# CompVis/behavior-driven-video-synthesis

Hardware: AMD Instinct MI355X
Metric: frames/sec VUnet 256x256 bs=16 fwd+bwd (higher is better)
Workload: dtype f32 (operands scaled by a power of two and split into 2 fp16 terms, 3 partial products on fp16 MFMA, fp32 accumulate; weight gradients and uncovered layers: 3 bf16 terms / 6 products, fp32-input MFMA, fp32 VALU); 1 GPU; Human3.6m shape_and_pose_net VunetAlter 256x256 per-GPU bs=16 fwd+bwd, VGG19 perceptual + KL loss, fused Adam, dropout 0.05, regressor side loop off, seeded-synthetic VGG19 weights, rasterised synthetic stickmen; global_batch=16, parallelism=dp1, conv_precision=h2, hip_streams=4, hip_graph=True, graph_settle_steps=7, rccl_world_size=1, dp_backend=none

## Files before the change

### behavior_driven_video_synthesis_amd/csrc/conv_wgrad_direct.hip

```cpp
#include <type_traits>

#include "common.h"
#include "split_h2.h"

struct WgradDirectArgs {
  vunet_wgrad_desc d;
  const float* x1;
  const float* x2;
  const float* dy;
  float* slabs;
  float* dshift;
  const float* amax_x;
  const float* amax_x2;
  const float* amax_dy;
  int Ctot, Coutp, ncot, noct, ops;
  int opr, opi;
  InAct in1, in2;
};

typedef uint32_t wd_u32x4 __attribute__((ext_vector_type(4)));
typedef float wd_f32x4 __attribute__((ext_vector_type(4)));

template <int S, bool W4, int T>
__device__ __forceinline__ void wgrad_direct_body(WgradDirectArgs& a, const int bx, const int by) {
  inact_resolve(a.in1);
  inact_resolve(a.in2);
  static_assert(T != 3 || !W4, "the kernel-row split is for maps >= 8 wide");
  constexpr int R = (T == 1 || T == 3) ? 1 : (W4 ? S + 3 : 3);
  constexpr int L = T == 1 ? 8 : (W4 ? 4 * S + 2 : 8 * S + 2);
  const vunet_wgrad_desc& d = a.d;
  const int tid = threadIdx.x, lane = tid & 63, wave = tid >> 6;
  const int j = lane & 31, h = lane >> 5;
  const int unit0 = bx * 4 + wave;
  const int krow = T == 3 ? unit0 % 3 : 0;
  const int unit = T == 3 ? unit0 / 3 : unit0;
  const int cot = unit % a.ncot, split = unit / a.ncot;
  const int ci0 = by * 32;
  const int H = d.Hs, W = d.Ws, HW = H * W, HoWo = d.Ho * d.Wo;

  float sx, sdy, descale, descale2;
  {
    __shared__ float redm[8];
    const float4 px = h2_amax4(a.amax_x, a.amax_x2, tid), pd = reinterpret_cast<const float4*>(a.amax_dy)[tid];
    float mx = wave_max(fmaxf(fmaxf(px.x, px.y), fmaxf(px.z, px.w)));
    float md = wave_max(fmaxf(fmaxf(pd.x, pd.y), fmaxf(pd.z, pd.w)));
    if (lane == 0) { redm[wave] = mx; redm[4 + wave] = md; }
    __syncthreads();
    mx = fmaxf(fmaxf(redm[0], redm[1]), fmaxf(redm[2], redm[3]));
    md = fmaxf(fmaxf(redm[4], redm[5]), fmaxf(redm[6], redm[7]));
    if (a.in1.thresh) mx *= a.in1.keep_scale;
    const int ex = h2_scale_exp(mx), ed = h2_scale_exp(md);
    sx = h2_pow2(ex);
    sdy = h2_pow2(ed);
    h2_pow2_pair(-(ex + ed), descale, descale2);
  }
  if (split >= d.nsplit) return;

  const int ci = ci0 + j;
  const bool ci_ok = ci < a.Ctot;
  const bool second = ci_ok && ci >= d.C1;
  const float* __restrict__ xs = second ? a.x2 : a.x1;
  const int Cs = second ? d.C2 : d.C1;
  const int cl = ci_ok ? (second ? ci - d.C1 : ci) : 0;
  InAct ia = a.in1;
  ia.seed = second ? a.in2.seed : a.in1.seed;
  const int co = cot * 32 + j;
  const bool co_ok = co < d.Cout;

  f32x16 acc[T];
#pragma unroll
  for (int t = 0; t < T; ++t)
#pragma unroll
    for (int r = 0; r < 16; ++r) acc[t][r] = 0.f;
  float dsum = 0.f;

  const int pro_form = in_act_form_of(a.in1);
  const int o_begin = split * a.ops, o_end = min(o_begin + a.ops, a.noct);
#pragma unroll(T == 1 ? 4 : 1)
  for (int o2 = o_begin; o2 < o_end; o2 += 2) {
    const int o = o2 + h;
    const bool ov = o < o_end;
    const int oc = ov ? o : o_begin;
    const int n = oc / a.opi, rem = oc - n * a.opi;
    int r0, c0;
    if (T == 1) { r0 = 0; c0 = rem * 8; }
    else if (W4) { r0 = rem * 2; c0 = 0; }
    else { r0 = rem / a.opr; c0 = (rem - r0 * a.opr) * 8; }

    h2_f16x8 Ah, Al;
    {
      const float* dp = a.dy + (size_t)(n * d.Cout + (co_ok ? co : 0)) * HoWo + (T == 1 ? c0 : r0 * d.Wo + c0);
      wd_f32x4 d0 = *reinterpret_cast<const wd_f32x4*>(dp), d1 = *reinterpret_cast<const wd_f32x4*>(dp + 4);
      if (!(ov && co_ok)) { d0 = wd_f32x4{0.f, 0.f, 0.f, 0.f}; d1 = d0; }
      dsum += ((d0[0] + d0[1]) + (d0[2] + d0[3])) + ((d1[0] + d1[1]) + (d1[2] + d1[3]));
      uint32_t ah[4], al[4];
      h2_split2_nat(d0[0] * sdy, d0[1] * sdy, ah[0], al[0]);
      h2_split2_nat(d0[2] * sdy, d0[3] * sdy, ah[1], al[1]);
      h2_split2_nat(d1[0] * sdy, d1[1] * sdy, ah[2], al[2]);
      h2_split2_nat(d1[2] * sdy, d1[3] * sdy, ah[3], al[3]);
      Ah = h2_frag(ah[0], ah[1], ah[2], ah[3]);
      Al = h2_frag(al[0], al[1], al[2], al[3]);
    }

    float seg[R][L];
    auto stage = [&](auto pro_c) {
      constexpr int PRO = decltype(pro_c)::value;
      const uint32_t cbase = (uint32_t)(n * Cs + cl) * (uint32_t)HW;
      const float* xp = xs + cbase;
#pragma unroll
      for (int rr = 0; rr < R; ++rr) {
        const int ih = T == 1 ? 0 : S * r0 - 1 + rr + krow;
        const bool rok = ov && ci_ok && (T == 1 || (unsigned)ih < (unsigned)H);
        const int ihc = rok ? ih : 0;
        const float sxr = rok ? sx : 0.f;
        if (T == 1) {
          const uint32_t off = (uint32_t)c0;
          const wd_f32x4 v0 = *reinterpret_cast<const wd_f32x4*>(xp + off), v1 = *reinterpret_cast<const wd_f32x4*>(xp + off + 4);
#pragma unroll
          for (int e = 0; e < 8; ++e) {
            const float t_ = e < 4 ? v0[e] : v1[e - 4];
            seg[rr][e] = in_act_form<PRO>(ia, rok ? t_ : 0.f, cbase + off + e) * sxr;
          }
        } else {
          constexpr int NV = (L - 2) / 4;
          const uint32_t off = (uint32_t)(ihc * W + S * c0);
          wd_f32x4 v[NV];
#pragma unroll
          for (int q = 0; q < NV; ++q) v[q] = *reinterpret_cast<const wd_f32x4*>(xp + off + 4 * q);
          const bool lok = rok && c0 > 0, hok = rok && S == 1 && S * c0 + 4 * NV < W;
          const float lv = xp[lok ? off - 1 : off];
          const float hv = xp[hok ? off + 4 * NV : off];
          seg[rr][0] = in_act_form<PRO>(ia, lok ? lv : 0.f, cbase + off - 1) * (lok ? sx : 0.f);
#pragma unroll
          for (int e = 0; e < 4 * NV; ++e)
            seg[rr][1 + e] = in_act_form<PRO>(ia, rok ? v[e >> 2][e & 3] : 0.f, cbase + off + e) * sxr;
          seg[rr][L - 1] = in_act_form<PRO>(ia, hok ? hv : 0.f, cbase + off + 4 * NV) * (hok ? sx : 0.f);
        }
      }
    };
    if (pro_form == 2) stage(std::integral_constant<int, 2>{});
    else if (pro_form == 1) stage(std::integral_constant<int, 1>{});
    else if (pro_form == 0) stage(std::integral_constant<int, 0>{});
    else stage(std::integral_constant<int, 3>{});

#pragma unroll
    for (int t = 0; t < T; ++t) {
      const int kh = T == 3 ? 0 : t / 3, kw = t % 3;
      float f[8];
#pragma unroll
      for (int e = 0; e < 8; ++e) {
        if (T == 1) f[e] = seg[0][e];
        else if (W4) f[e] = seg[(e >> 2) * S + kh][(e & 3) * S + kw];
        else f[e] = seg[kh][e * S + kw];
      }
      uint32_t bh[4], bl[4];
      h2_split2_nat(f[0], f[1], bh[0], bl[0]);
      h2_split2_nat(f[2], f[3], bh[1], bl[1]);
      h2_split2_nat(f[4], f[5], bh[2], bl[2]);
      h2_split2_nat(f[6], f[7], bh[3], bl[3]);
      const h2_f16x8 Bh = h2_frag(bh[0], bh[1], bh[2], bh[3]), Bl = h2_frag(bl[0], bl[1], bl[2], bl[3]);
      f32x16 cc = acc[t];
      cc = __builtin_amdgcn_mfma_f32_32x32x16_f16(Ah, Bl, cc, 0, 0, 0);
      cc = __builtin_amdgcn_mfma_f32_32x32x16_f16(Al, Bh, cc, 0, 0, 0);
      cc = __builtin_amdgcn_mfma_f32_32x32x16_f16(Ah, Bh, cc, 0, 0, 0);
      acc[t] = cc;
    }
  }

  const size_t KT = (size_t)(T == 3 ? 9 : T) * a.Ctot;
  float* slab = a.slabs + (size_t)split * a.Coutp * KT;
  if (ci_ok) {
    auto store = [&](auto tc) {
      constexpr int t = decltype(tc)::value;
      const int tap = T == 3 ? krow * 3 + t : t;
#pragma unroll
      for (int r = 0; r < 16; ++r) {
        const int cr = cot * 32 + (r & 3) + 8 * (r >> 2) + 4 * h;
        if (cr < d.Cout) slab[(size_t)cr * KT + (size_t)tap * a.Ctot + ci] = acc[t][r] * descale * descale2;
      }
    };
    store(std::integral_constant<int, 0>{});
    if constexpr (T == 3) {
      store(std::integral_constant<int, 1>{});
      store(std::integral_constant<int, 2>{});
    }
    if constexpr (T == 9) {
      store(std::integral_constant<int, 1>{});
      store(std::integral_constant<int, 2>{});
      store(std::integral_constant<int, 3>{});
      store(std::integral_constant<int, 4>{});
      store(std::integral_constant<int, 5>{});
      store(std::integral_constant<int, 6>{});
      store(std::integral_constant<int, 7>{});
      store(std::integral_constant<int, 8>{});
    }
  }
  if (by == 0 && krow == 0) {
    const float tot = dsum + __shfl_xor(dsum, 32, 64);
    if (h == 0 && co < a.Coutp) a.dshift[(size_t)split * a.Coutp + co] = co_ok ? tot : 0.f;
  }
}

template <int S, bool W4, int T>
__global__ __launch_bounds__(256, 2) void conv_wgrad_direct_kernel(const WgradDirectArgs a_in) {
  WgradDirectArgs a = a_in;
  wgrad_direct_body<S, W4, T>(a, (int)blockIdx.x, (int)blockIdx.y);
}

struct S2Lds {
  static constexpr int PITCH = 48;
  static constexpr int XPLANE = 32 * PITCH;
  static constexpr int XBYTES = 3 * 4 * XPLANE;
  static constexpr int DYCOT = 2 * 32 * PITCH;
};

__device__ __forceinline__ wd_f32x4 s2_load4(const float* p) {
  wd_f32x4 v;
  asm volatile("global_load_dwordx4 %0, %1, off" : "=v"(v) : "v"(p) : "memory");
  return v;
}
__device__ __forceinline__ float s2_load1(const float* p) {
  float v;
  asm volatile("global_load_dword %0, %1, off" : "=v"(v) : "v"(p) : "memory");
  return v;
}
template <int N>
__device__ __forceinline__ void s2_wait() {
  static_assert(N >= 0 && N < 64, "vmcnt is six bits");
  asm volatile("s_waitcnt vmcnt(%0)" ::"n"(N) : "memory");
}

template <int NWAVE, int NU, int NCOT>
__global__ __launch_bounds__(64 * NWAVE) void conv_wgrad_s2_kernel(const WgradDirectArgs a_in) {
  WgradDirectArgs a = a_in;
  inact_resolve(a.in1);
  inact_resolve(a.in2);
  constexpr int NTHR = 64 * NWAVE;
  constexpr int NX = (3 * 32 * 8 + NTHR - 1) / NTHR;
  constexpr int NDY = (NCOT * 32 * 4 + NTHR - 1) / NTHR;
  extern __shared__ __attribute__((aligned(16))) unsigned char s2_lds[];
  unsigned char* const xL = s2_lds;
  unsigned char* const dL = s2_lds + S2Lds::XBYTES;
  const vunet_wgrad_desc& d = a.d;
  const int tid = threadIdx.x, lane = tid & 63, wave = tid >> 6;
  const int j = lane & 31, h = lane >> 5;
  const int split = blockIdx.x, ci0 = blockIdx.y * 32;
  const int H = d.Hs, W = d.Ws, HW = H * W, HoWo = d.Ho * d.Wo;
  const int ppr = d.Wo >> 4, ppi = d.Ho * ppr;

  float sx, sdy, descale, descale2;
  {
    __shared__ float redm[2 * NWAVE];
    float mx = 0.f, md = 0.f;
    for (int i = tid; i < 256; i += NTHR) {
      const float4 px = h2_amax4(a.amax_x, a.amax_x2, i), pd = reinterpret_cast<const float4*>(a.amax_dy)[i];
      mx = fmaxf(mx, fmaxf(fmaxf(px.x, px.y), fmaxf(px.z, px.w)));
      md = fmaxf(md, fmaxf(fmaxf(pd.x, pd.y), fmaxf(pd.z, pd.w)));
    }
    mx = wave_max(mx);
    md = wave_max(md);
    if (lane == 0) { redm[wave] = mx; redm[NWAVE + wave] = md; }
    __syncthreads();
    mx = md = 0.f;
#pragma unroll
    for (int w = 0; w < NWAVE; ++w) { mx = fmaxf(mx, redm[w]); md = fmaxf(md, redm[NWAVE + w]); }
    if (a.in1.thresh) mx *= a.in1.keep_scale;
    const int ex = h2_scale_exp(mx), ed = h2_scale_exp(md);
    sx = h2_pow2(ex);
    sdy = h2_pow2(ed);
    h2_pow2_pair(-(ex + ed), descale, descale2);
  }
  const bool second = ci0 >= d.C1;
  const float* __restrict__ xs = second ? a.x2 : a.x1;
  const int Cs = second ? d.C2 : d.C1, cl0 = second ? ci0 - d.C1 : ci0;
  InAct ia = a.in1;
  ia.seed = second ? a.in2.seed : a.in1.seed;
  const int pro_form = in_act_form_of(a.in1);

  const int pairs = d.N * ppi, pps = (pairs + d.nsplit - 1) / d.nsplit;
  const int pb = split * pps, pe = min(pb + pps, pairs);

  const int krow = wave % 3, cotb = wave / 3;
  f32x16 acc[NU][3];
#pragma unroll
  for (int u = 0; u < NU; ++u)
#pragma unroll
    for (int t = 0; t < 3; ++t)
// ... 156 lines not shown
      for (int i = 0; i < NX; ++i) asm volatile("" : "+v"(xv[K_][i]) : : "memory");
#pragma unroll
      for (int i = 0; i < NDY; ++i) asm volatile("" : "+v"(dv[K_][i]) : : "memory");
      asm volatile("" : "+v"(xhalo[K_]) : : "memory");
    }
    lds_barrier();
    if (pro_form == 2) convert(p, std::integral_constant<int, 2>{}, slot_c);
    else if (pro_form == 1) convert(p, std::integral_constant<int, 1>{}, slot_c);
    else if (pro_form == 0) convert(p, std::integral_constant<int, 0>{}, slot_c);
    else convert(p, std::integral_constant<int, 3>{}, slot_c);
    lds_barrier();
    if (p + D < pe) prefetch(p + D, slot_c);
    if (cotb < NCOT) multiply();
  };
  if (pb + 0 < pe) prefetch(pb + 0, std::integral_constant<int, 0>{});
  if constexpr (D == 4) {
    if (pb + 1 < pe) prefetch(pb + 1, std::integral_constant<int, 1>{});
    if (pb + 2 < pe) prefetch(pb + 2, std::integral_constant<int, 2>{});
    if (pb + 3 < pe) prefetch(pb + 3, std::integral_constant<int, 3>{});
  }
  for (int p0 = pb; p0 < pe; p0 += D) {
    step(p0, std::integral_constant<int, 0>{});
    if constexpr (D == 4) {
      if (p0 + 1 < pe) step(p0 + 1, std::integral_constant<int, 1>{});
      if (p0 + 2 < pe) step(p0 + 2, std::integral_constant<int, 2>{});
      if (p0 + 3 < pe) step(p0 + 3, std::integral_constant<int, 3>{});
    }
  }

  const size_t KT = (size_t)9 * a.Ctot;
  float* slab = a.slabs + (size_t)split * a.Coutp * KT;
#pragma unroll
  for (int u = 0; u < NU; ++u) {
    const int cot = cotb + 2 * u;
    if (cot >= NCOT) continue;
#pragma unroll
    for (int t = 0; t < 3; ++t)
#pragma unroll
      for (int r = 0; r < 16; ++r) {
        const int cr = cot * 32 + (r & 3) + 8 * (r >> 2) + 4 * h;
        slab[(size_t)cr * KT + (size_t)(krow * 3 + t) * a.Ctot + ci0 + j] = acc[u][t][r] * descale * descale2;
      }
  }
  if (blockIdx.y == 0) {
#pragma unroll
    for (int i = 0; i < NDY; ++i) {
      const int u = tid + NTHR * i;
      const int q4 = u & 3, co = (u >> 2) & 31, cot = u >> 7;
      float t = dsum[i];
      t += __shfl_xor(t, 1, 64);
      t += __shfl_xor(t, 2, 64);
      if (q4 == 0 && cot < NCOT) a.dshift[(size_t)split * a.Coutp + cot * 32 + co] = t;
    }
  }
}

static bool s2_staged_ok(const vunet_wgrad_desc* d) {
  if (g_vunet_tune[VUNET_TUNE_WGRAD_ROWSPLIT] == 3) return false;
  if (!(d->flags & 2) || (d->flags & 1)) return false;
  if (d->KH != 3 || d->KW != 3 || d->stride != 2 || d->pad != 1) return false;
  if (d->Ws != 2 * d->Wo || d->Hs != 2 * d->Ho || d->Wo % 16) return false;
  if (d->C1 % 32 || d->C2 % 32 || d->Cout % 32) return false;
  const int ncot = d->Cout / 32;
  if (ncot != 1 && ncot != 2 && ncot != 4) return false;
  return (int64_t)d->N * d->Ho * d->Wo > 16384;
}

static int s2_staged_nslabs(const vunet_wgrad_desc* d) {
  const int ncit = (d->C1 + d->C2) / 32, pairs = d->N * d->Ho * (d->Wo / 16);
  int S = 512 / ncit;
  if (S > pairs / 4) S = pairs / 4;
  return S < 1 ? 1 : S;
}

constexpr int WD_MULTI = 12;
struct WgradDirectBatch {
  WgradDirectArgs it[WD_MULTI];
  int start[WD_MULTI + 1];
  int gx[WD_MULTI];
  int n;
};
static_assert(sizeof(WgradDirectBatch) <= 4096, "kernel arguments: 4 KB");
template <int S, bool W4, int T>
__global__ __launch_bounds__(256, 2) void conv_wgrad_direct_multi_kernel(const WgradDirectBatch b) {
  int i = 0;
  while (i + 1 < b.n && (int)blockIdx.x >= b.start[i + 1]) ++i;
  WgradDirectArgs a = b.it[i];
  const int local = (int)blockIdx.x - b.start[i];
  wgrad_direct_body<S, W4, T>(a, local % b.gx[i], local / b.gx[i]);
}

static int direct_class(const vunet_wgrad_desc* d) {
  if (!(d->flags & 2) || (d->flags & 1)) return 0;
  if (d->C1 <= 0 || d->Cout <= 0 || (d->C2 > 0 && d->C1 % 32 != 0)) return 0;
  if (d->Cout < 16 && d->KH == 3) return 0;
  if (d->KH == 1 && d->KW == 1) {
    if (d->stride != 1 || d->pad != 0 || d->Ho != d->Hs || d->Wo != d->Ws || (d->Hs * d->Ws) % 8) return 0;
    return 1;
  }
  if (d->KH != 3 || d->KW != 3 || d->pad != 1 || (d->stride != 1 && d->stride != 2)) return 0;
  if (d->Ho != (d->Hs - 1) / d->stride + 1 || d->Wo != (d->Ws - 1) / d->stride + 1) return 0;
  if (d->Ws % 4) return 0;
  if (d->Wo == 4 && d->Ws == 4 * d->stride && d->Ho % 2 == 0) return d->stride == 1 ? 2 : 3;
  if (d->Wo % 8 == 0 && d->Ws == d->Wo * d->stride) return d->stride == 1 ? 4 : 5;
  return 0;
}

bool vunet_wgrad_direct_applicable(const vunet_wgrad_desc* d) { return direct_class(d) != 0; }

static void direct_geometry(const vunet_wgrad_desc* d, WgradDirectArgs& a) {
  const int cls = direct_class(d);
  a.Ctot = d->C1 + d->C2;
  a.Coutp = (d->Cout + 31) / 32 * 32;
  a.ncot = a.Coutp / 32;
  if (cls == 1) { a.opr = 0; a.opi = d->Hs * d->Ws / 8; }
  else if (cls == 2 || cls == 3) { a.opr = 0; a.opi = d->Ho / 2; }
  else { a.opr = d->Wo / 8; a.opi = d->Ho * a.opr; }
  a.noct = d->N * a.opi;
}

static bool direct_rowsplit(int cls) {
  const int knob = g_vunet_tune[VUNET_TUNE_WGRAD_ROWSPLIT];
  if (knob == 1) return false;
  return cls == 5 || (knob != 4 && cls == 4);
}

int vunet_wgrad_direct_nslabs(const vunet_wgrad_desc* d) {
  if (s2_staged_ok(d)) return s2_staged_nslabs(d);
  WgradDirectArgs a;
  direct_geometry(d, a);
  const int ncit = (a.Ctot + 31) / 32;
  int S = 2048 / (a.ncot * ncit * (direct_rowsplit(direct_class(d)) ? 3 : 1));
  const int by_work = (a.noct + 7) / 8;
  if (S > by_work) S = by_work;
  if (S < 1) S = 1;
  const int cap = d->KH == 1 ? 2048 : 512;
  if (S > cap) S = cap;
  return S;
}

int vunet_wgrad_direct_name(const vunet_wgrad_desc* d, char* name, int len) {
  if (s2_staged_ok(d)) return snprintf(name, len, "conv_wgrad_s2_kernel");
  const int cls = direct_class(d);
  const int S = (cls == 3 || cls == 5) ? 2 : 1, W4 = (cls == 2 || cls == 3), T = cls == 1 ? 1 : (direct_rowsplit(cls) ? 3 : 9);
  return snprintf(name, len, "conv_wgrad_direct_kernel<%d, %s, %d>", S, W4 ? "true" : "false", T);
}

static void direct_fill(const vunet_wgrad_desc* d, const float* x1, const float* x2, const float* dy, float* slabs, float* dshift,
                        const float* amax_x, const float* amax_x2, const float* amax_dy, WgradDirectArgs& a, int& gx, int& gy) {
  a.d = *d;
  a.x1 = x1; a.x2 = x2; a.dy = dy; a.slabs = slabs; a.dshift = dshift; a.amax_x = amax_x; a.amax_x2 = amax_x2; a.amax_dy = amax_dy;
  direct_geometry(d, a);
  a.ops = (a.noct + d->nsplit - 1) / d->nsplit;
  a.ops = (a.ops + 1) & ~1;
  a.in1 = make_inact(d->in_act, d->in_slope, d->drop_p, d->drop_seed);
  a.in2 = make_inact(d->in_act, d->in_slope, d->drop_p, d->drop_seed + 0x9E3779B9u);
  const int units = d->nsplit * a.ncot * (direct_rowsplit(direct_class(d)) ? 3 : 1);
  gx = (units + 3) / 4;
  gy = (a.Ctot + 31) / 32;
}

static int direct_form(const vunet_wgrad_desc* d) {
  const int cls = direct_class(d);
  return cls ? cls * 2 + (direct_rowsplit(cls) ? 1 : 0) : 0;
}

template <int S, bool W4, int T>
static void direct_launch_batch(const WgradDirectBatch& b, hipStream_t st) {
  VUNET_LAUNCH((conv_wgrad_direct_multi_kernel<S, W4, T>), dim3((unsigned)b.start[b.n]), dim3(256), 0, st, b);
}

int vunet_wgrad_direct_launch_multi(const vunet_wgrad_item* items, const int* idx, int cnt, hipStream_t st) {
  if (cnt < 1) return VUNET_OK;
  const int form = direct_form(&items[idx[0]].d);
  if (!form) return VUNET_ERR_UNSUPPORTED;
  for (int at = 0; at < cnt; at += WD_MULTI) {
    WgradDirectBatch b;
    b.n = cnt - at < WD_MULTI ? cnt - at : WD_MULTI;
    b.start[0] = 0;
    for (int k = 0; k < b.n; ++k) {
      const vunet_wgrad_item& it = items[idx[at + k]];
      if (direct_form(&it.d) != form) return VUNET_ERR_ARG;
      if (!it.x1 || !it.dy || !it.slabs || !it.dshift || !it.amax_x || !it.amax_dy || (it.d.C2 > 0 && !it.x2)) return VUNET_ERR_ARG;
      int gx, gy;
      direct_fill(&it.d, it.x1, it.x2, it.dy, it.slabs, it.dshift, it.amax_x, it.amax_x2, it.amax_dy, b.it[k], gx, gy);
      b.gx[k] = gx;
      b.start[k + 1] = b.start[k] + gx * gy;
    }
    for (int k = b.n; k < WD_MULTI; ++k) { b.it[k] = b.it[0]; b.gx[k] = 1; b.start[k + 1] = b.start[b.n]; }
    switch (form) {
      case 2: direct_launch_batch<1, false, 1>(b, st); break;
      case 4: direct_launch_batch<1, true, 9>(b, st); break;
      case 6: direct_launch_batch<2, true, 9>(b, st); break;
      case 8: direct_launch_batch<1, false, 9>(b, st); break;
      case 9: direct_launch_batch<1, false, 3>(b, st); break;
      case 10: direct_launch_batch<2, false, 9>(b, st); break;
      case 11: direct_launch_batch<2, false, 3>(b, st); break;
      default: return VUNET_ERR_UNSUPPORTED;
    }
    const int rc = vunet_check_launch();
    if (rc != VUNET_OK) return rc;
  }
  return VUNET_OK;
}

int vunet_wgrad_direct_form(const vunet_wgrad_desc* d) { return direct_form(d); }

int vunet_wgrad_direct_launch(const vunet_wgrad_desc* d, const float* x1, const float* x2, const float* dy, float* slabs,
                              float* dshift, const float* amax_x, const float* amax_x2, const float* amax_dy, hipStream_t st) {
  const int cls = direct_class(d);
  if (!cls) return VUNET_ERR_UNSUPPORTED;
  WgradDirectArgs a;
  int gx, gy;
  direct_fill(d, x1, x2, dy, slabs, dshift, amax_x, amax_x2, amax_dy, a, gx, gy);
  if (s2_staged_ok(d)) {
    const int ncot = d->Cout / 32;
    dim3 grid((unsigned)d->nsplit, (unsigned)((d->C1 + d->C2) / 32));
    const size_t lds = (size_t)S2Lds::XBYTES + (size_t)ncot * S2Lds::DYCOT;
    if (ncot == 1) VUNET_LAUNCH((conv_wgrad_s2_kernel<3, 1, 1>), grid, dim3(192), lds, st, a);
    else if (ncot == 2) VUNET_LAUNCH((conv_wgrad_s2_kernel<6, 1, 2>), grid, dim3(384), lds, st, a);
    else VUNET_LAUNCH((conv_wgrad_s2_kernel<6, 2, 4>), grid, dim3(384), lds, st, a);
    return vunet_check_launch();
  }
  const bool rs = direct_rowsplit(cls);
  dim3 grid((unsigned)gx, (unsigned)gy), block(256);
  if (rs) {
    if (cls == 5) VUNET_LAUNCH((conv_wgrad_direct_kernel<2, false, 3>), grid, block, 0, st, a);
    else VUNET_LAUNCH((conv_wgrad_direct_kernel<1, false, 3>), grid, block, 0, st, a);
    return vunet_check_launch();
  }
  switch (cls) {
    case 1: VUNET_LAUNCH((conv_wgrad_direct_kernel<1, false, 1>), grid, block, 0, st, a); break;
    case 2: VUNET_LAUNCH((conv_wgrad_direct_kernel<1, true, 9>), grid, block, 0, st, a); break;
    case 3: VUNET_LAUNCH((conv_wgrad_direct_kernel<2, true, 9>), grid, block, 0, st, a); break;
    case 4: VUNET_LAUNCH((conv_wgrad_direct_kernel<1, false, 9>), grid, block, 0, st, a); break;
    default: VUNET_LAUNCH((conv_wgrad_direct_kernel<2, false, 9>), grid, block, 0, st, a); break;
  }
  return vunet_check_launch();
}
```

### behavior_driven_video_synthesis_amd/ops.py

```python
from __future__ import annotations

import contextlib
import ctypes
import os
from dataclasses import dataclass
from typing import Optional, Tuple

import torch

from . import _lib

ACT_NONE, ACT_ELU, ACT_RELU, ACT_SIGMOID, ACT_LRELU = 0, 1, 2, 3, 4
SEED2_OFFSET = 0x9E3779B9


class ConvDesc(ctypes.Structure):
    _fields_ = [("N", ctypes.c_int32), ("C1", ctypes.c_int32), ("C2", ctypes.c_int32), ("Hs", ctypes.c_int32),
                ("Ws", ctypes.c_int32), ("M", ctypes.c_int32), ("m_off", ctypes.c_int32), ("Mpad", ctypes.c_int32),
                ("Ho", ctypes.c_int32), ("Wo", ctypes.c_int32), ("KH", ctypes.c_int32), ("KW", ctypes.c_int32),
                ("stride", ctypes.c_int32), ("pad", ctypes.c_int32), ("mode", ctypes.c_int32),
                ("in_act", ctypes.c_int32), ("in_slope", ctypes.c_float), ("drop_p", ctypes.c_float),
                ("drop_seed", ctypes.c_uint32), ("out_act", ctypes.c_int32), ("d2s", ctypes.c_int32),
                ("aux_act", ctypes.c_int32), ("aux_slope", ctypes.c_float), ("aux_drop_p", ctypes.c_float),
                ("aux_drop_seed", ctypes.c_uint32)]
# ... 61 lines not shown
def _r32(x: int) -> int:
    return (x + 31) // 32 * 32


_drop_state = {"base": None, "ctr": 0, "step": None, "host_step": 0}


def set_dropout_seed(seed: int):
    _drop_state["base"] = int(seed) & 0xFFFFFFFF
    _drop_state["ctr"] = 0


def set_dropout_host_step(step: int):
    _drop_state["host_step"] = int(step) & 0xFFFFFFFF


def reset_dropout_counter():
    if _drop_state["base"] is None:
        set_dropout_seed(torch.initial_seed())
    _drop_state["ctr"] = 0


def set_dropout_step(counter: Optional[torch.Tensor]):
    if counter is not None and not (counter.is_cuda and counter.dtype == torch.int32 and counter.numel() == 1):
        raise RuntimeError("dropout step counter: one int32 element on the GPU")
    _drop_state["step"] = counter
    _call("vunet_set_dropout_step", _p(counter))


def dropout_step_counter() -> Optional[torch.Tensor]:
    return _drop_state["step"]


def next_dropout_seed() -> int:
    if _drop_state["base"] is None:
        set_dropout_seed(torch.initial_seed())
    _drop_state["ctr"] += 1
    x = (_drop_state["base"] * 0x9E3779B1 + _drop_state["ctr"] * 0x85EBCA77) & 0xFFFFFFFF
    x ^= x >> 15
    return ((x * 0x2C1B3C6D) + _drop_state["host_step"] * 0x9E3779B1) & 0xFFFFFFFF


@dataclass
class ConvCfg:
    kind: int = 0
    k: int = 3
    stride: int = 1
    pad: int = 0
    in_act: int = ACT_NONE
    in_slope: float = 0.0
    drop_p: float = 0.0
    drop_seed: int = 0
    out_act: int = ACT_NONE
    d2s: bool = False
    res_is_x1: bool = False
    owner: object = None
    bf16: bool = False
    passthrough: bool = False


def conv_out_size(h: int, k: int, stride: int, pad: int) -> int:
    return (h + 2 * pad - k) // stride + 1


_SCHEMES = {"f32": 0, "x6": 1, "h2": 2}
_conv_precision = {"mode": os.environ.get("VUNET_CONV_SCHEME", "h2")}


def set_conv_precision(mode: str):
    if mode not in _SCHEMES:
        raise ValueError(f"unknown conv precision {mode!r} (h2 | x6 | f32)")
    _conv_precision["mode"] = mode


def conv_precision() -> str:
    return _conv_precision["mode"]


def _scheme() -> int:
    return _SCHEMES[_conv_precision["mode"]]


_wants_split_cache = {}
_TUNING_KEYS = {"split_force_nt": 0, "tiled_force_nt": 1, "force_small": 2, "blk_force_nt": 3, "parity_launches": 4, "blk_ws": 5, "wgrad_rowsplit": 6, "s2_fwd_f32": 7, "p2_form": 8}


def set_tuning(key: str, value: int):
    _call("vunet_set_tuning", _TUNING_KEYS[key], int(value))
    _wants_split_cache.clear()


def apply_env_tuning():
    spec = os.environ.get("VUNET_TUNING", "")
    for kv in filter(None, (t.strip() for t in spec.split(","))):
        k, _, v = kv.partition("=")
        set_tuning(k.strip(), int(v))


def absmax_partials(x1, x2=None):
    out = torch.empty(1024, device=x1.device, dtype=torch.float32)
    _call("vunet_absmax_partials", _p(x1), x1.numel(), _p(x2), 0 if x2 is None else x2.numel(), _p(out), _stream())
    return out


_amax_arena = {}


def _new_amax_out(dev):
    idx = dev.index if dev.index is not None else torch.cuda.current_device()
    key = (idx, _raw_stream(idx) if _raw_stream is not None else 0)
    a = _amax_arena.get(key)
    if a is None or a[1] >= a[0].shape[0]:
        a = _amax_arena[key] = [torch.zeros(128, 1024, device=dev, dtype=torch.float32), 0]
    a[1] += 1
    return a[0][a[1] - 1]


def _zero_scalar(dev, shape=(1,)):
    idx = dev.index if dev.index is not None else torch.cuda.current_device()
    key = (idx, _raw_stream(idx) if _raw_stream is not None else 0)
    z = _zero_rows.get(key)
    if z is None or z[1] + 16 > z[0].numel():
        z = _zero_rows[key] = [_new_amax_out(dev), 0]
    z[1] += 16
    return z[0][z[1] - 16:z[1] - 15].view(shape)


_zero_rows = {}
_amax_retired = []


def _reset_amax_arena():
    _amax_retired[:] = [list(_amax_arena.values())]
    _amax_arena.clear()
    _zero_rows.clear()


def _tag_amax(t, buf):
    t._vunet_amax = (buf, t._version)


def _tagged_amax(t):
    rec = getattr(t, "_vunet_amax", None)
    return rec[0] if rec is not None and rec[1] == t._version else None


def carry_amax_tag(src, dst):
    tag = _tagged_amax(src)
    if tag is not None:
        _tag_amax(dst, tag)
    if _is_relu_out(src):
        _tag_relu_out(dst)


_relu_premask = os.environ.get("VUNET_RELU_PREMASK", "1") != "0"


def enable_relu_premask(on: bool = True):
    global _relu_premask
    _relu_premask = bool(on)


def _tag_relu_out(t):
    t._vunet_relu_out = t._version


def _is_relu_out(t) -> bool:
# ... 1488 lines not shown
```

### include/vunet_hip.h

```cpp
#ifndef VUNET_HIP_H
#define VUNET_HIP_H
#include <stddef.h>
#include <stdint.h>

#ifdef __cplusplus
extern "C" {
#endif

#define VUNET_OK 0
#define VUNET_ERR_ARG (-1)
#define VUNET_ERR_LAUNCH (-2)
#define VUNET_ERR_UNSUPPORTED (-3)

#define VUNET_ACT_NONE 0
#define VUNET_ACT_ELU 1
#define VUNET_ACT_RELU 2
#define VUNET_ACT_SIGMOID 3
#define VUNET_ACT_LRELU 4

int vunet_abi_version(void);

typedef struct vunet_conv_desc {
  int32_t N;
  int32_t C1, C2;
// ... 116 lines not shown

int vunet_weightnorm_bwd(const vunet_wn_desc* d, const float* slabs, const float* dshift, int32_t nsplit,
                         const float* v, const float* g, const float* bias, const float* gamma,
                         const float* invnorm, float* dv, float* dg, float* dbias, float* dgamma,
                         float* dbeta, float* workspace, int32_t accumulate, void* stream);

typedef struct vunet_wn_bwd_item {
  const float *slabs, *dshift, *v, *g, *bias, *gamma, *invnorm;
  float *dv, *dg, *dbias, *dgamma, *dbeta;
  float* workspace;
  vunet_wn_desc d;
  int32_t nsplit, accumulate;
} vunet_wn_bwd_item;
int vunet_weightnorm_bwd_multi(const vunet_wn_bwd_item* items_dev, int32_t n_items, int32_t max_cout,
                               int32_t max_reduce_blocks, void* stream);

int vunet_depth_to_space(const float* x, float* y, int32_t N, int32_t C, int32_t H, int32_t W, void* stream);
int vunet_space_to_depth(const float* x, float* y, int32_t N, int32_t C, int32_t H, int32_t W, void* stream);

int vunet_upsample_bilinear2x_fwd(const float* x, float* y, int64_t NC, int32_t H, int32_t W, void* stream);
int vunet_upsample_bilinear2x_bwd(const float* dy, float* dx, int64_t NC, int32_t H, int32_t W, void* stream);

int vunet_axpby(const float* x, const float* y_in, float* y, float a, float b, int64_t n, void* stream);
int vunet_act_bwd_from_out(const float* y, const float* dy, float* dx, int32_t act, float slope, int64_t n,
                           void* stream);
int vunet_act_fwd(const float* x, float* y, int32_t act, float slope, int64_t n, void* stream);

int vunet_reparam_fwd(const float* mu, const float* logstd, const float* eps, float* z, int64_t n, void* stream);
int vunet_reparam_bwd(const float* dz, const float* logstd, const float* eps, float* dmu, float* dlogstd,
                      int64_t n, void* stream);

int vunet_l1_mean_fwd(const float* a, const float* b, float* partial, float* out, float weight, int64_t n,
                      void* stream);
int vunet_l1_mean_bwd(const float* a, const float* b, const float* add, float* db, float gscale,
                      const float* gout, int64_t n, void* stream);
int vunet_l1_mean_bwd_amax(const float* a, const float* b, const float* add, float* db, float gscale,
                           const float* gout, int64_t n, float* amax_out, int32_t relu_mask, void* stream);

int vunet_kl_fwd(const float* mu, const float* logstd, float* partial, float* out, float weight, int32_t N, int64_t D,
                 void* stream);
int vunet_kl_bwd(const float* mu, const float* logstd, float* dmu, float* dlogstd, float gscale,
                 const float* gout, int64_t n, void* stream);
int vunet_sqdiff_fwd(const float* p, const float* q, float* partial, float* out, float weight, int32_t N, int64_t D,
                     void* stream);
int vunet_sqdiff_bwd(const float* p, const float* q, float* dp, float* dq, float gscale, const float* gout,
                     int64_t n, void* stream);

int vunet_vgg_preprocess(const float* x, float* y, int32_t N, int32_t H, int32_t W, void* stream);
int vunet_vgg_preprocess_bwd(const float* dy, const float* add, float* dx, int32_t N, int32_t H, int32_t W,
                             void* stream);
int vunet_maxpool2_fwd(const float* x, float* y, int32_t NC, int32_t H, int32_t W, void* stream);
int vunet_l1_pool_fwd(const float* a, const float* b, float* partial, float* out, float* y, float weight, int32_t NC,
                      int32_t H, int32_t W, void* stream);
int vunet_l1_pool_bwd(const float* a, const float* b, const float* dy_pool, float* db, float gscale, const float* gout,
                      int32_t NC, int32_t H, int32_t W, float* amax_out, int32_t relu_mask, void* stream);
int vunet_maxpool2_bwd_relu(const float* x, const float* y, const float* dy, float* dx, int32_t NC, int32_t H, int32_t W,
                            void* stream);
int vunet_maxpool2_bwd(const float* x, const float* y, const float* dy, float* dx, int32_t NC, int32_t H,
                       int32_t W, void* stream);

int vunet_instnorm_fwd(const float* x, float* y, float* stats, int32_t NC, int32_t HW, float eps, void* stream);
int vunet_instnorm_bwd(const float* y, const float* dy, const float* stats, float* dx, int32_t NC, int32_t HW,
                       void* stream);

int vunet_adam_step(float* param, const float* grad, float* exp_avg, float* exp_avg_sq, int64_t n, float lr,
                    float beta1, float beta2, float eps, float weight_decay, int32_t step, float grad_scale,
                    void* stream);

int vunet_adam_step_dev(float* param, const float* grad, float* exp_avg, float* exp_avg_sq, int64_t n,
                        const double* lr_dev, float beta1, float beta2, float eps, float weight_decay,
                        const int64_t* step_dev, float grad_scale, void* stream);

int vunet_set_dropout_step(const uint32_t* step_dev);

#define VUNET_TUNE_SPLIT_FORCE_NT 0
#define VUNET_TUNE_TILED_FORCE_NT 1
#define VUNET_TUNE_FORCE_SMALL 2
#define VUNET_TUNE_BLK_FORCE_NT 3
#define VUNET_TUNE_PARITY_LAUNCHES 4
#define VUNET_TUNE_BLK_WS 5
#define VUNET_TUNE_WGRAD_ROWSPLIT 6
#define VUNET_TUNE_S2_FWD_F32 7
#define VUNET_TUNE_P2_FORM 8
#define VUNET_TUNE_COUNT 9
int vunet_set_tuning(int32_t key, int32_t value);

int vunet_dropout_mask(float* mask, int64_t n, float p, uint32_t seed, void* stream);

int vunet_stickman_raster(const float* kps, int32_t B, int32_t J, const int32_t* body, int32_t n_body,
                          const int32_t* cmds, int32_t n_cmds, uint8_t* out_u8, float* out_f32, int32_t H, int32_t W,
                          void* stream);
int vunet_stickman_raster_thick(const float* kps, int32_t B, int32_t J, const int32_t* body, int32_t n_body,
                                const int32_t* cmds, int32_t n_cmds, uint8_t* out_u8, float* out_f32, int32_t H, int32_t W,
                                int32_t thickness, void* stream);
int vunet_u8_to_unit(const uint8_t* in, float* out, int64_t n, void* stream);

int vunet_ssim_partial(const float* x, const float* y, int32_t planes, int32_t H, int32_t W, float data_range,
                       const float* window11, float* partial, void* stream);

int vunet_dp_available(void);
int vunet_dp_unique_id(void* id128);
int vunet_dp_init(int32_t world, int32_t rank, const void* id128);
int vunet_dp_world(void);
int vunet_dp_allreduce_bucket(float* buf, int64_t n, int32_t average, void* stream);
int vunet_dp_finalize(void);

int vunet_crop_window(const float* x, float* y, int32_t planes, int32_t H, int32_t W, int32_t P, const int32_t* off,
                      void* stream);
int vunet_crop_window_bwd(const float* dy, float* dx, int32_t planes, int32_t H, int32_t W, int32_t P, const int32_t* off,
                          void* stream);

#define VUNET_LOSS_MAX_TERMS 8
int vunet_total_loss(const float* const* terms, int32_t n, const float* kl, const float* gamma, float gamma_const,
                     float ll_weight, int32_t use_kl, float* loss, float* ll, void* stream);
int vunet_total_loss_bwd(const float* g_loss, const float* g_ll, int32_t n, const float* gamma, float gamma_const,
                         float ll_weight, int32_t use_kl, float* d, void* stream);
int vunet_gamma_update(float* gamma, const float* imax, const float* avg_kl, float gamma_step, void* stream);

int vunet_unit_sample(const float* mu, const float* logstd, float* z, float* eps_out, int64_t n, uint32_t seed, void* stream);

int vunet_set_schedule(double* lr_dev, double lr, float* imax_dev, float imax, int32_t* step_dev, int32_t step, void* stream);

int vunet_sum_amax(const float* const* srcs, int32_t n, float* out, float* amax_out, int64_t numel, void* stream);

typedef struct vunet_p2_desc {
  int32_t N, C, H, W;
  int32_t M;
  int32_t relu;
} vunet_p2_desc;
int vunet_p2_conv_supported(const vunet_p2_desc* d);
int vunet_p2_conv_variant(const vunet_p2_desc* d, char* name, int32_t len);
int vunet_p2_conv(const vunet_p2_desc* d, const void* x, const int32_t* xmeta, const void* w_image, const float* wk,
                  const float* shift, const void* mask, void* y, int32_t* ymeta, void* stream);
int vunet_p2_weight_image_bytes(int32_t Cout, int32_t Cin, int32_t dgrad);
int vunet_p2_pack_weights(const float* w, const float* shift, int32_t Cout, int32_t Cin, int32_t dgrad, void* image, float* wk,
                          float* workspace, void* stream);
int vunet_p2_weight_bound(const float* w, const float* shift, int32_t Cout, int32_t Cin, float* wk, float* workspace, void* stream);
int vunet_p2_conv_first(const float* x, const float* amax_x, int32_t n_amax, const float* wt_f, int32_t Mpad, const float* shift,
                        const float* wk, void* y, int32_t* ymeta, int32_t N, int32_t H, int32_t W, int32_t M, void* stream);
int vunet_p2_from_nchw(const float* x, const float* amax, int32_t n_amax, int32_t relu, void* y, int32_t* ymeta, int32_t N,
                       int32_t C, int32_t H, int32_t W, void* stream);
int vunet_p2_to_nchw(const void* x, const int32_t* xmeta, float* y, int32_t N, int32_t C, int32_t H, int32_t W, void* stream);

int vunet_p2_l1_fwd(const void* t, const int32_t* tmeta, const void* p, const int32_t* pmeta, float* partial, float* out,
                    float weight, int32_t N, int32_t C, int32_t H, int32_t W, void* stream);
int vunet_p2_pool_fwd(const void* t, const int32_t* tmeta, const void* p, const int32_t* pmeta, float* partial, float* out,
                      float weight, void* y, int32_t* ymeta, int32_t N, int32_t C, int32_t H, int32_t W, void* stream);
int vunet_p2_l1_bwd(const void* t, const int32_t* tmeta, const void* p, const int32_t* pmeta, const void* add,
                    const int32_t* addmeta, void* g, int32_t* gmeta, float gscale, const float* gout, int32_t N, int32_t C,
                    int32_t H, int32_t W, void* stream);
int vunet_p2_pool_bwd(const void* t, const int32_t* tmeta, const void* p, const int32_t* pmeta, const void* dy,
                      const int32_t* dymeta, void* g, int32_t* gmeta, float gscale, const float* gout, int32_t N, int32_t C,
                      int32_t H, int32_t W, void* stream);

typedef struct vunet_seq_linear_desc {
  int32_t B, M, K, ldx, act0, act1, nets, shared_in, S;
} vunet_seq_linear_desc;
typedef struct vunet_seq_coupling_desc {
  int32_t B, C, c1, ld_in, ld_out, Mp, reverse, affine_on_src, S;
} vunet_seq_coupling_desc;
typedef struct vunet_seq_lstm_desc {
  int32_t B, H, ldx, hoff, n, ldraw;
  int64_t seq_stride;
} vunet_seq_lstm_desc;
int vunet_seq_linear(const vunet_seq_linear_desc* d, const float* w0, const float* w1, const float* x, const float* bias0,
                     const float* bias1, float* y, void* stream);
int vunet_seq_coupling(const vunet_seq_coupling_desc* d, const float* in, const float* st, const float* bias_s, const float* bias_t,
// ... 25 lines not shown
```

Measured before the change: 800.1 frames/s.

## Fold wgrad split-K partials inside a block via LDS reduction

Adds a tunable fold factor so that 2 or 4 waves in a block share one split-K unit, each covering a sub-range of output tiles, and reduce their accumulators through shared memory before one wave writes the slab. This cuts the number of global slab partials and the downstream reduction traffic. The launch bounds for non-9-tap variants are also raised to 4 blocks per CU, which may constrain register allocation. The fold defaults to 1 because the tuning knob is zero unless set, so only the launch-bounds change and the readfirstlane on the wave index affect the default path.

```diff
diff --git a/behavior_driven_video_synthesis_amd/csrc/conv_wgrad_direct.hip b/behavior_driven_video_synthesis_amd/csrc/conv_wgrad_direct.hip
--- a/behavior_driven_video_synthesis_amd/csrc/conv_wgrad_direct.hip
+++ b/behavior_driven_video_synthesis_amd/csrc/conv_wgrad_direct.hip
@@ -14,6 +14,7 @@
   const float* amax_x2;
   const float* amax_dy;
   int Ctot, Coutp, ncot, noct, ops;
+  int fold;
   int opr, opi;
   InAct in1, in2;
 };
@@ -29,9 +30,11 @@
   constexpr int R = (T == 1 || T == 3) ? 1 : (W4 ? S + 3 : 3);
   constexpr int L = T == 1 ? 8 : (W4 ? 4 * S + 2 : 8 * S + 2);
   const vunet_wgrad_desc& d = a.d;
-  const int tid = threadIdx.x, lane = tid & 63, wave = tid >> 6;
+  const int tid = threadIdx.x, lane = tid & 63;
+  const int wave = __builtin_amdgcn_readfirstlane(tid >> 6);
   const int j = lane & 31, h = lane >> 5;
-  const int unit0 = bx * 4 + wave;
+  const int F = a.fold, fs = F >> 1;
+  const int unit0 = bx * (4 >> fs) + (wave >> fs), sub = wave & (F - 1);
   const int krow = T == 3 ? unit0 % 3 : 0;
   const int unit = T == 3 ? unit0 / 3 : unit0;
   const int cot = unit % a.ncot, split = unit / a.ncot;
@@ -54,7 +57,8 @@
     sdy = h2_pow2(ed);
     h2_pow2_pair(-(ex + ed), descale, descale2);
   }
-  if (split >= d.nsplit) return;
+  if (F == 1 && split >= d.nsplit) return;
+  const bool live = split < d.nsplit;
 
   const int ci = ci0 + j;
   const bool ci_ok = ci < a.Ctot;
@@ -75,7 +79,7 @@
   float dsum = 0.f;
 
   const int pro_form = in_act_form_of(a.in1);
-  const int o_begin = split * a.ops, o_end = min(o_begin + a.ops, a.noct);
+  const int o_begin = live ? (split * F + sub) * a.ops : 0, o_end = live ? min(o_begin + a.ops, a.noct) : 0;
 #pragma unroll(T == 1 ? 4 : 1)
   for (int o2 = o_begin; o2 < o_end; o2 += 2) {
     const int o = o2 + h;
@@ -167,6 +171,35 @@
     }
   }
 
+  if (F > 1) {
+    __shared__ wd_f32x4 fold_acc[3][4][64];
+    __shared__ float fold_ds[3][64];
+    const int slot0 = (wave >> fs) * (F - 1);
+    if (sub > 0) fold_ds[slot0 + sub - 1][lane] = dsum;
+#pragma unroll
+    for (int t = 0; t < T; ++t) {
+      if (sub > 0) {
+#pragma unroll
+        for (int q = 0; q < 4; ++q)
+          fold_acc[slot0 + sub - 1][q][lane] = wd_f32x4{acc[t][4 * q], acc[t][4 * q + 1], acc[t][4 * q + 2], acc[t][4 * q + 3]};
+      }
+      __syncthreads();
+      if (sub == 0) {
+        for (int s = 0; s < F - 1; ++s) {
+#pragma unroll
+          for (int q = 0; q < 4; ++q) {
+            const wd_f32x4 v = fold_acc[slot0 + s][q][lane];
+#pragma unroll
+            for (int e = 0; e < 4; ++e) acc[t][4 * q + e] += v[e];
+          }
+        }
+      }
+      __syncthreads();
+    }
+    if (sub > 0 || !live) return;
+    for (int s = 0; s < F - 1; ++s) dsum += fold_ds[slot0 + s][lane];
+  }
+
   const size_t KT = (size_t)(T == 3 ? 9 : T) * a.Ctot;
   float* slab = a.slabs + (size_t)split * a.Coutp * KT;
   if (ci_ok) {
@@ -202,7 +235,7 @@
 }
 
 template <int S, bool W4, int T>
-__global__ __launch_bounds__(256, 2) void conv_wgrad_direct_kernel(const WgradDirectArgs a_in) {
+__global__ __launch_bounds__(256, T == 9 ? 2 : 4) void conv_wgrad_direct_kernel(const WgradDirectArgs a_in) {
   WgradDirectArgs a = a_in;
   wgrad_direct_body<S, W4, T>(a, (int)blockIdx.x, (int)blockIdx.y);
 }
@@ -525,7 +558,7 @@
 };
 static_assert(sizeof(WgradDirectBatch) <= 4096, "kernel arguments: 4 KB");
 template <int S, bool W4, int T>
-__global__ __launch_bounds__(256, 2) void conv_wgrad_direct_multi_kernel(const WgradDirectBatch b) {
+__global__ __launch_bounds__(256, T == 9 ? 2 : 4) void conv_wgrad_direct_multi_kernel(const WgradDirectBatch b) {
   int i = 0;
   while (i + 1 < b.n && (int)blockIdx.x >= b.start[i + 1]) ++i;
   WgradDirectArgs a = b.it[i];
@@ -568,8 +601,7 @@
   return cls == 5 || (knob != 4 && cls == 4);
 }
 
-int vunet_wgrad_direct_nslabs(const vunet_wgrad_desc* d) {
-  if (s2_staged_ok(d)) return s2_staged_nslabs(d);
+static int direct_nsplit_unfolded(const vunet_wgrad_desc* d) {
   WgradDirectArgs a;
   direct_geometry(d, a);
   const int ncit = (a.Ctot + 31) / 32;
@@ -582,6 +614,18 @@
   return S;
 }
 
+static int direct_fold(const vunet_wgrad_desc* d) {
+  (void)d;
+  const int knob = g_vunet_tune[VUNET_TUNE_WGRAD_FOLD];
+  return (knob == 2 || knob == 4) ? knob : 1;
+}
+
+int vunet_wgrad_direct_nslabs(const vunet_wgrad_desc* d) {
+  if (s2_staged_ok(d)) return s2_staged_nslabs(d);
+  const int F = direct_fold(d);
+  return (direct_nsplit_unfolded(d) + F - 1) / F;
+}
+
 int vunet_wgrad_direct_name(const vunet_wgrad_desc* d, char* name, int len) {
   if (s2_staged_ok(d)) return snprintf(name, len, "conv_wgrad_s2_kernel");
   const int cls = direct_class(d);
@@ -594,12 +638,15 @@
   a.d = *d;
   a.x1 = x1; a.x2 = x2; a.dy = dy; a.slabs = slabs; a.dshift = dshift; a.amax_x = amax_x; a.amax_x2 = amax_x2; a.amax_dy = amax_dy;
   direct_geometry(d, a);
-  a.ops = (a.noct + d->nsplit - 1) / d->nsplit;
+  a.fold = direct_fold(d);
+  const int nsub = d->nsplit * a.fold;
+  a.ops = (a.noct + nsub - 1) / nsub;
   a.ops = (a.ops + 1) & ~1;
   a.in1 = make_inact(d->in_act, d->in_slope, d->drop_p, d->drop_seed);
   a.in2 = make_inact(d->in_act, d->in_slope, d->drop_p, d->drop_seed + 0x9E3779B9u);
   const int units = d->nsplit * a.ncot * (direct_rowsplit(direct_class(d)) ? 3 : 1);
-  gx = (units + 3) / 4;
+  const int upw = 4 / a.fold;
+  gx = (units + upw - 1) / upw;
   gy = (a.Ctot + 31) / 32;
 }
 
diff --git a/behavior_driven_video_synthesis_amd/ops.py b/behavior_driven_video_synthesis_amd/ops.py
--- a/behavior_driven_video_synthesis_amd/ops.py
+++ b/behavior_driven_video_synthesis_amd/ops.py
@@ -167,7 +167,7 @@
 
 
 _wants_split_cache = {}
-_TUNING_KEYS = {"split_force_nt": 0, "tiled_force_nt": 1, "force_small": 2, "blk_force_nt": 3, "parity_launches": 4, "blk_ws": 5, "wgrad_rowsplit": 6, "s2_fwd_f32": 7, "p2_form": 8}
+_TUNING_KEYS = {"split_force_nt": 0, "tiled_force_nt": 1, "force_small": 2, "blk_force_nt": 3, "parity_launches": 4, "blk_ws": 5, "wgrad_rowsplit": 6, "s2_fwd_f32": 7, "p2_form": 8, "wgrad_fold": 9}
 
 
 def set_tuning(key: str, value: int):
diff --git a/include/vunet_hip.h b/include/vunet_hip.h
--- a/include/vunet_hip.h
+++ b/include/vunet_hip.h
@@ -222,7 +222,8 @@
 #define VUNET_TUNE_WGRAD_ROWSPLIT 6
 #define VUNET_TUNE_S2_FWD_F32 7
 #define VUNET_TUNE_P2_FORM 8
-#define VUNET_TUNE_COUNT 9
+#define VUNET_TUNE_WGRAD_FOLD 9
+#define VUNET_TUNE_COUNT 10
 int vunet_set_tuning(int32_t key, int32_t value);
 
 int vunet_dropout_mask(float* mask, int64_t n, float p, uint32_t seed, void* stream);
```

Measured after the change: 800.5 frames/s, median of 2. No clear change (+0.1%).
